# UCL/gp_emulator

Measured on AMD Instinct MI355X. Metric: test-points/sec for predict(mean+var+grad), N_train=250 D=11, higher is better.
Workload: dtype f64

## Files before the change

### gp_emulator_amd/csrc/gp_ctx.hip

```cpp
#include "gp_host.hpp"

#include <cstdarg>
#include <cstdio>

#include "gp_launchers.hpp"
#include "gp_train_args.hpp"

static thread_local char g_err[512] = "";

int fail(int code, const char* fmt, ...) {
  va_list ap;
  va_start(ap, fmt);
  vsnprintf(g_err, sizeof(g_err), fmt, ap);
  va_end(ap);
  return code;
}

int check_call(const gp_ctx* ctx, const gp_model* model, int64_t n) {
  if (!ctx || !model) return fail(GP_ERR_INVALID, "null context or model");
  if (n < 0) return fail(GP_ERR_INVALID, "n_predict < 0");
  return GP_OK;
}
int check_layout(int deriv_layout) {
  if (deriv_layout == GP_DERIV_DMAJOR || deriv_layout == GP_DERIV_ROWMAJOR) return GP_OK;
// ... 64 lines not shown
    return fail(GP_ERR_HIP, "hipStreamCreate: %s", hipGetErrorString(e));
  }
  e = hipMalloc((void**)&c->tickets, 4 * kTicketSlots * sizeof(unsigned));
  if (e == hipSuccess) e = hipMemset(c->tickets, 0, 4 * kTicketSlots * sizeof(unsigned));
  if (e != hipSuccess) {
    if (c->tickets) (void)hipFree(c->tickets);
    (void)hipStreamDestroy(c->stream);
    delete c;
    return fail(GP_ERR_HIP, "context item counters: %s", hipGetErrorString(e));
  }
  *out = c;
  return GP_OK;
}

int gp_ctx_destroy(gp_ctx* ctx) {
  if (!ctx) return GP_OK;
  (void)hipSetDevice(ctx->device);
  (void)hipStreamSynchronize(ctx->stream);
  for (auto& c : ctx->cache)
    if (c.model) gp_model_destroy(c.model);
  if (ctx->scratch) (void)hipFree(ctx->scratch);
  if (ctx->tickets) (void)hipFree(ctx->tickets);
  gp_pipe& pp = ctx->pipe;
  pp.pool.reset();
  for (int k = 0; k < kPipeSlots; ++k) {
    if (pp.stream[k]) (void)hipStreamSynchronize(pp.stream[k]);
    if (pp.stage_in[k]) (void)hipHostFree(pp.stage_in[k]);
    if (pp.stage_out[k]) (void)hipHostFree(pp.stage_out[k]);
    if (pp.dev[k]) (void)hipFree(pp.dev[k]);
    if (pp.done[k]) (void)hipEventDestroy(pp.done[k]);
    if (pp.in_there[k]) (void)hipEventDestroy(pp.in_there[k]);
    if (pp.computed[k]) (void)hipEventDestroy(pp.computed[k]);
    if (pp.stream[k]) (void)hipStreamDestroy(pp.stream[k]);
  }
  if (pp.up) { (void)hipStreamSynchronize(pp.up); (void)hipStreamDestroy(pp.up); }
  if (pp.down) { (void)hipStreamSynchronize(pp.down); (void)hipStreamDestroy(pp.down); }
  (void)hipStreamDestroy(ctx->stream);
  delete ctx;
  return GP_OK;
}

int gp_ctx_set_debug_buffer(gp_ctx* ctx, void* d_buffer) {
  if (!ctx) return fail(GP_ERR_INVALID, "null context");
  ctx->dbg = d_buffer;
  return GP_OK;
}

int gp_ctx_synchronize(gp_ctx* ctx) {
  if (!ctx) return fail(GP_ERR_INVALID, "null context");
  HIP_TRY(hipSetDevice(ctx->device));
  HIP_TRY(hipStreamSynchronize(ctx->stream));
  return GP_OK;
}

int gp_ctx_device_info(gp_ctx* ctx, int* compute_units, int64_t* hbm_bytes, char* name, int name_len) {
  if (!ctx) return fail(GP_ERR_INVALID, "null context");
// ... 148 lines not shown
```

### gp_emulator_amd/csrc/gp_host.hpp

```cpp
#pragma once
#include "gp_predict_hip.h"

#include <hip/hip_runtime.h>
#include <atomic>
#include <cstdlib>
#include <cstring>
#include <exception>
#include <memory>
#include <mutex>
#include <new>
#include <vector>

#include "gp_dispatch.hpp"
#include "gp_host_pool.hpp"
#include "gp_predict_kernel.hpp"

#pragma GCC visibility push(hidden)

int fail(int code, const char* fmt, ...) __attribute__((format(printf, 2, 3)));

template <typename F>
static int guarded(F&& body) noexcept {
  try {
    return body();
  } catch (const std::bad_alloc&) {
    return fail(GP_ERR_NOMEM, "out of host memory");
  } catch (const std::exception& ex) {
    return fail(GP_ERR_INVALID, "%s", ex.what());
  } catch (...) {
    return fail(GP_ERR_INVALID, "unknown C++ exception");
  }
}

#define HIP_TRY(expr)                                                                 \
  do {                                                                                \
    hipError_t e_ = (expr);                                                           \
    if (e_ != hipSuccess)                                                             \
// ... 21 lines not shown
template <typename T> constexpr int dtype_of() { return sizeof(T) == 8 ? GP_F64 : GP_F32; }

struct gp_model {
  int device;
  int dtype;
  int n_train, n_inputs;
  int kernel_d, kernel_nb;
  int kernel_nk;
  int n_emulators;
  long long xa_stride, frags_stride, sd_stride;
  void* d_xa;
  void* d_frags;
  void* d_sd;
  std::vector<double> scale_host, centre_host;
  std::vector<double> xs_host;
  std::mutex h_mutex;
  void* d_pfrags;
  long long pfrags_stride;
  void* d_vfrags;
  long long vfrags_stride;
};

constexpr int kPipeSlotsMax = 6;
inline int pipe_slots() {
  static const int n = [] {
    const char* ev = getenv("GP_HOST_SLOTS");
    const int v = ev ? atoi(ev) : 3;
    return v < 2 ? 2 : (v > kPipeSlotsMax ? kPipeSlotsMax : v);
  }();
  return n;
}
#define kPipeSlots pipe_slots()
struct gp_pipe {
  bool ready = false;
  hipStream_t stream[kPipeSlotsMax] = {};
  hipEvent_t done[kPipeSlotsMax] = {};
  hipStream_t up = nullptr, down = nullptr;
  hipEvent_t in_there[kPipeSlotsMax] = {}, computed[kPipeSlotsMax] = {};
  void* stage_in[kPipeSlotsMax] = {};
  void* stage_out[kPipeSlotsMax] = {};
  void* dev[kPipeSlotsMax] = {};

  size_t stage_in_bytes = 0, stage_out_bytes = 0, dev_bytes = 0;
  std::unique_ptr<gph::ThreadPool> pool;
};

struct gp_cached_model {
  gp_model* model = nullptr;
  int host_dtype = 0, compute_dtype = 0, n_train = 0, n_inputs = 0, theta_size = 0;
  bool with_invq = false;
  std::vector<char> key;
  unsigned long long stamp = 0;
};
constexpr int kModelCacheSlots = 4;

static const int kTicketSlots = 256;

struct gp_ctx {
  int device;
  hipStream_t stream;
  int compute_units;
  void* scratch;
  size_t scratch_bytes;
  void* dbg;
  unsigned* tickets = nullptr;
  std::atomic<unsigned> ticket_next{0};
  gp_pipe pipe;
// ... 51 lines not shown
```

### gp_emulator_amd/csrc/gp_host_path.hip

```cpp
#include "gp_host.hpp"

#include <cctype>
#include <chrono>
#include <cstdio>

#include <sched.h>

static int device_numa_node(int device) {
  char bdf[64] = "";
  if (hipDeviceGetPCIBusId(bdf, (int)sizeof(bdf), device) != hipSuccess) return -1;
  for (char* c = bdf; *c; ++c) *c = (char)tolower(*c);
  char path[160];
  snprintf(path, sizeof(path), "/sys/bus/pci/devices/%s/numa_node", bdf);
  FILE* fh = fopen(path, "r");
  if (!fh) return -1;
  int node = -1;
  if (fscanf(fh, "%d", &node) != 1) node = -1;
  fclose(fh);
  return node;
}
static bool node_cpus(int node, cpu_set_t* out) {
  CPU_ZERO(out);
  if (node < 0) return false;
  char path[96];
// ... 20 lines not shown
  static int n = [] {
    int avail = 1;
    cpu_set_t set;
    CPU_ZERO(&set);
    if (sched_getaffinity(0, sizeof(set), &set) == 0) avail = CPU_COUNT(&set);
    const char* ev = getenv("GP_HOST_THREADS");
    int v = ev ? atoi(ev) : 8;
    if (v > avail) v = avail;
    return v < 1 ? 1 : (v > 32 ? 32 : v);
  }();
  return n;
}

gph::ThreadPool& host_pool(gp_ctx* ctx) {
  if (!ctx->pipe.pool) {
    cpu_set_t cpus;
    const char* ev = getenv("GP_HOST_PIN");
    const bool pin = (!ev || atoi(ev) != 0) && node_cpus(device_numa_node(ctx->device), &cpus);
    ctx->pipe.pool.reset(new gph::ThreadPool(host_threads(), pin ? &cpus : nullptr));
  }
  return *ctx->pipe.pool;
}

static int ensure_pipe(gp_ctx* ctx, size_t in_bytes, size_t out_bytes, size_t dev_only_bytes = 0) {
  gp_pipe& pp = ctx->pipe;
  if (!pp.ready) {
    for (int k = 0; k < kPipeSlots; ++k) {
      if (!pp.stream[k]) HIP_TRY(hipStreamCreateWithFlags(&pp.stream[k], hipStreamNonBlocking));
      if (!pp.done[k]) HIP_TRY(hipEventCreateWithFlags(&pp.done[k], hipEventDisableTiming));
      if (!pp.in_there[k]) HIP_TRY(hipEventCreateWithFlags(&pp.in_there[k], hipEventDisableTiming));
      if (!pp.computed[k]) HIP_TRY(hipEventCreateWithFlags(&pp.computed[k], hipEventDisableTiming));
    }
    if (!pp.up) HIP_TRY(hipStreamCreateWithFlags(&pp.up, hipStreamNonBlocking));
    if (!pp.down) HIP_TRY(hipStreamCreateWithFlags(&pp.down, hipStreamNonBlocking));
    pp.ready = true;
  }
  auto host_alloc = [&](void** slot, size_t bytes) -> hipError_t {
    hipError_t err = hipSuccess;
    const int dev = ctx->device;
    host_pool(ctx).run_on_worker([&] {
      err = hipSetDevice(dev);
      if (err == hipSuccess) err = hipHostMalloc(slot, bytes, hipHostMallocDefault);
      if (err == hipSuccess) std::memset(*slot, 0, bytes);
    });
    return err;
  };
  if (dev_only_bytes == 0 && pp.stage_in_bytes < in_bytes) {
    pp.stage_in_bytes = 0;
    for (int k = 0; k < kPipeSlots; ++k) {
      if (pp.stage_in[k]) { void* q = pp.stage_in[k]; pp.stage_in[k] = nullptr; HIP_TRY(hipHostFree(q)); }
      HIP_TRY(host_alloc(&pp.stage_in[k], in_bytes));
    }
    pp.stage_in_bytes = in_bytes;
  }
  if (dev_only_bytes == 0 && pp.stage_out_bytes < out_bytes) {
    pp.stage_out_bytes = 0;
    for (int k = 0; k < kPipeSlots; ++k) {
      if (pp.stage_out[k]) { void* q = pp.stage_out[k]; pp.stage_out[k] = nullptr; HIP_TRY(hipHostFree(q)); }
      HIP_TRY(host_alloc(&pp.stage_out[k], out_bytes));
    }
    pp.stage_out_bytes = out_bytes;
  }
  const size_t dev_need = dev_only_bytes ? dev_only_bytes : in_bytes + out_bytes;
  if (pp.dev_bytes < dev_need) {
    pp.dev_bytes = 0;
    for (int k = 0; k < kPipeSlots; ++k) {
      if (pp.dev[k]) { void* q = pp.dev[k]; pp.dev[k] = nullptr; HIP_TRY(hipFree(q)); }
      HIP_TRY(hipMalloc(&pp.dev[k], dev_need));
    }
    pp.dev_bytes = dev_need;
  }
  return GP_OK;
}

template <typename T>
static int64_t slab_rows(const gp_ctx* ctx, const gp_model* m, int64_t M, int64_t out_row_elems, int64_t max_rows) {
  constexpr int64_t kRowsPerWG = gpk::Geo<T>::kRowsPerWG;
  static const int rounds = [] { const char* ev = getenv("GP_HOST_SLAB_ROUNDS"); const int v = ev ? atoi(ev) : 2; return v < 1 ? 1 : v; }();
  int64_t slab = rounds * (int64_t)ctx->compute_units * gpk::Geo<T>::kWGPerCU * kRowsPerWG;
  const int64_t by_bytes = ((int64_t)(m->n_emulators > 1 ? 64 : 16) << 20) / (int64_t)(out_row_elems * sizeof(T));
  if (slab > by_bytes) slab = by_bytes;
  if (M < 4 * slab && M >= 4 * 8192) slab = (M + 3) / 4;
  slab = (slab + kRowsPerWG - 1) / kRowsPerWG * kRowsPerWG;
  if (max_rows > 0 && slab > max_rows) slab = max_rows;
  if (slab > M) slab = M;
  return slab < 1 ? 1 : slab;
}

template <typename T, typename FIn, typename FLaunch, typename FOut>
static int run_slab_pipeline(gp_ctx* ctx, int64_t M, int64_t slab, size_t in_row, size_t out_row,
                             FIn copy_in, FLaunch launch, FOut copy_out) {
  const size_t in_elems = (size_t)slab * in_row, out_elems = (size_t)slab * out_row;
  int rc = ensure_pipe(ctx, in_elems * sizeof(T), out_elems * sizeof(T));
  if (rc) return rc;
  gp_pipe& pp = ctx->pipe;
  const int64_t ns = (M + slab - 1) / slab;
  auto rows_of = [&](int64_t s) { return (s + 1) * slab <= M ? slab : M - s * slab; };
  auto tasks_for = [&](int64_t n, size_t row_bytes) {
    const size_t bytes = (size_t)n * row_bytes;
    int t = (int)(bytes / ((size_t)256 << 10));
    const int cap = 2 * host_threads();
    return t < 1 ? 1 : (t > cap ? cap : t);
  };
  static const bool trace = [] { const char* ev = getenv("GP_HOST_TRACE"); return ev && atoi(ev) != 0; }();
  auto now = [] { return std::chrono::steady_clock::now(); };
  double t_wait = 0, t_copy = 0, t_enq = 0;
  const auto t_begin = now();
  hipError_t e = hipSuccess;
  for (int64_t s = 0; s < ns + kPipeSlots && e == hipSuccess && rc == GP_OK; ++s) {
    const int k = (int)(s % kPipeSlots);
    const int64_t so = s - kPipeSlots;
    const bool has_out = so >= 0 && so < ns, has_in = s < ns;
    if (!has_out && !has_in) continue;
    const int64_t n_out = has_out ? rows_of(so) : 0, n_in = has_in ? rows_of(s) : 0;
    auto t0 = now();
    if (has_out) {
      e = hipEventSynchronize(pp.done[k]);
      if (e != hipSuccess) break;
    }
    auto t1 = now();
    const int t_out = has_out ? tasks_for(n_out, out_row * sizeof(T)) : 0;
    const int t_in = has_in ? tasks_for(n_in, in_row * sizeof(T)) : 0;
    const T* o_stage = (const T*)pp.stage_out[k];
    T* i_stage = (T*)pp.stage_in[k];
    auto task = [&](int t) {
      if (t < t_in) {
        const int64_t lo = n_in * t / t_in, hi = n_in * (t + 1) / t_in;
        copy_in(i_stage, s * slab, n_in, lo, hi);
      } else {
        const int u = t - t_in;
        const int64_t lo = n_out * u / t_out, hi = n_out * (u + 1) / t_out;
        copy_out(o_stage, so * slab, n_out, lo, hi);
      }
    };
    const int n_tasks = t_in + t_out;
    static const int skip_host = [] { const char* ev = getenv("GP_HOST_SKIP"); return ev ? atoi(ev) & 8 : 0; }();
    if (skip_host) {}
    else if (n_tasks == 1) task(0);
    else host_pool(ctx).run(n_tasks, task);
    auto t2 = now();
    if (has_in) {
      static const int skip = [] { const char* ev = getenv("GP_HOST_SKIP"); return ev ? atoi(ev) : 0; }();
      T* d_in = (T*)pp.dev[k];
      T* d_out = d_in + in_elems;
      static const int dir_streams = [] { const char* ev = getenv("GP_PIPE_DIRSTREAMS"); return ev ? atoi(ev) : 3; }();
      const bool own_up = dir_streams & 1, own_down = dir_streams & 2;
      hipStream_t s_up = own_up ? pp.up : pp.stream[k], s_down = own_down ? pp.down : pp.stream[k];
      if (!(skip & 1))
        e = hipMemcpyAsync(d_in, pp.stage_in[k], sizeof(T) * (size_t)n_in * in_row, hipMemcpyHostToDevice, s_up);
      if (e != hipSuccess) break;
      if (own_up) {
        e = hipEventRecord(pp.in_there[k], s_up);
        if (e == hipSuccess) e = hipStreamWaitEvent(pp.stream[k], pp.in_there[k], 0);
        if (e != hipSuccess) break;
      }
      if (!(skip & 2)) rc = launch(d_in, d_out, n_in, pp.stream[k]);
      if (rc) break;
      if (own_down) {
        e = hipEventRecord(pp.computed[k], pp.stream[k]);
        if (e == hipSuccess) e = hipStreamWaitEvent(s_down, pp.computed[k], 0);
        if (e != hipSuccess) break;
      }
      if (!(skip & 4))
        e = hipMemcpyAsync(pp.stage_out[k], d_out, sizeof(T) * (size_t)n_in * out_row, hipMemcpyDeviceToHost, s_down);
      if (e == hipSuccess) e = hipEventRecord(pp.done[k], s_down);
    }
    if (trace) {
      auto t3 = now();
      t_wait += std::chrono::duration<double>(t1 - t0).count();
      t_copy += std::chrono::duration<double>(t2 - t1).count();
      t_enq += std::chrono::duration<double>(t3 - t2).count();
    }
  }
  for (int k = 0; k < kPipeSlots; ++k) (void)hipStreamSynchronize(pp.stream[k]);
  (void)hipStreamSynchronize(pp.up);
  (void)hipStreamSynchronize(pp.down);
  if (trace)
    fprintf(stderr, "[gp host pipeline] rows=%lld slab=%lld slabs=%lld threads=%d: total %.3f ms = event waits %.3f + host copies %.3f + enqueue %.3f\n",
            (long long)M, (long long)slab, (long long)ns, host_threads(),
            std::chrono::duration<double>(now() - t_begin).count() * 1e3, t_wait * 1e3, t_copy * 1e3, t_enq * 1e3);
  if (rc) return rc;
  if (e != hipSuccess) return fail(GP_ERR_HIP, "host pipeline: %s", hipGetErrorString(e));
  return GP_OK;
}

static bool is_pinned_host(const void* p, size_t bytes) {
  if (!p) return false;
  hipPointerAttribute_t a;
  if (hipPointerGetAttributes(&a, p) != hipSuccess) { (void)hipGetLastError(); return false; }
  if (a.type != hipMemoryTypeHost) return false;
  hipPointerAttribute_t b;
  if (hipPointerGetAttributes(&b, (const char*)p + (bytes ? bytes - 1 : 0)) != hipSuccess) { (void)hipGetLastError(); return false; }
  return b.type == hipMemoryTypeHost;
}

template <typename T>
static int predict_host_pinned(gp_ctx* ctx, const gp_model* m, const T* testing, T* result, T* error, T* deriv,
                               int64_t M, int64_t max_rows) {
  const int D = m->n_inputs;
  constexpr int64_t kRowsPerWG = gpk::Geo<T>::kRowsPerWG;
  const int64_t round = (int64_t)ctx->compute_units * gpk::Geo<T>::kWGPerCU * kRowsPerWG;
  int64_t cap = 4 * round;
  if (max_rows > 0 && cap > max_rows) cap = max_rows < kRowsPerWG ? kRowsPerWG : max_rows / kRowsPerWG * kRowsPerWG;
  const bool want_var = error != nullptr;
  const size_t in_elems = (size_t)cap * D, out_elems = (size_t)cap * ((want_var ? 2 : 1) + D);
  int rc = ensure_pipe(ctx, 0, 0, (in_elems + out_elems) * sizeof(T));
  if (rc) return rc;
  gp_pipe& pp = ctx->pipe;
  hipError_t e = hipSuccess;
  int64_t s0 = 0, cur = round < cap ? round : cap;
  for (int64_t s = 0; s0 < M && e == hipSuccess && rc == GP_OK; ++s) {
    const int k = (int)(s % kPipeSlots);
    const int64_t n = s0 + cur <= M ? cur : M - s0;
    if (s >= kPipeSlots) e = hipEventSynchronize(pp.done[k]);
    if (e != hipSuccess) break;
    T* d_in = (T*)pp.dev[k];
    T* d_mu = d_in + in_elems;
    T* d_var = want_var ? d_mu + n : nullptr;
    T* d_der = d_mu + (want_var ? 2 : 1) * n;
    e = hipMemcpyAsync(d_in, testing + (size_t)s0 * D, sizeof(T) * (size_t)n * D, hipMemcpyHostToDevice, pp.up);
    if (e == hipSuccess) e = hipEventRecord(pp.in_there[k], pp.up);
    if (e == hipSuccess) e = hipStreamWaitEvent(pp.stream[k], pp.in_there[k], 0);
    if (e != hipSuccess) break;
    rc = predict_device<T>(ctx, m, d_in, d_mu, d_var, d_der, n, GP_DERIV_ROWMAJOR, pp.stream[k]);
    if (rc) break;
    e = hipEventRecord(pp.computed[k], pp.stream[k]);
    if (e == hipSuccess) e = hipStreamWaitEvent(pp.down, pp.computed[k], 0);
    if (e == hipSuccess) e = hipMemcpyAsync(deriv + (size_t)s0 * D, d_der, sizeof(T) * (size_t)n * D, hipMemcpyDeviceToHost, pp.down);
    if (e == hipSuccess) e = hipMemcpyAsync(result + s0, d_mu, sizeof(T) * (size_t)n, hipMemcpyDeviceToHost, pp.down);
// ... 81 lines not shown
                             layout, st, prescale);
  };
  auto copy_out = [=](const T* o, int64_t s0, int64_t n, int64_t lo, int64_t hi) {
    int e_lo = 0, e_hi = E;
    if (E > 1) {
      e_lo = (int)((int64_t)E * lo / n);
      e_hi = (int)((int64_t)E * hi / n);
      lo = 0;
      hi = n;
    }
    for (int e = e_lo; e < e_hi; ++e) {
      convert_range(result + (size_t)e * M + s0, o + (size_t)e * n, (size_t)lo, (size_t)hi);
      if (want_var) convert_range(error + (size_t)e * M + s0, o + (size_t)(E + e) * n, (size_t)lo, (size_t)hi);
      const T* od = o + (size_t)nv * E * n + (size_t)e * n * D;
      TH* hd = deriv + (size_t)e * M * D;
      if (layout == GP_DERIV_ROWMAJOR) {
        convert_range(hd + (size_t)s0 * D, od, (size_t)lo * D, (size_t)hi * D);
      } else {
        for (int d = 0; d < D; ++d)
          convert_range(hd + (size_t)d * M + s0, od + (size_t)d * n, (size_t)lo, (size_t)hi);
      }
    }
  };
  return run_slab_pipeline<T>(ctx, M, slab, (size_t)D, out_row, copy_in, launch, copy_out);
}

template <typename T, typename TH = T>
static int hessian_host_model(gp_ctx* ctx, const gp_model* m, const TH* testing, TH* hess, int64_t M) {
  const int D = m->n_inputs, E = m->n_emulators;
  if (M == 0) return GP_OK;
  HIP_TRY(hipSetDevice(ctx->device));
  const size_t dd = (size_t)D * D;
  const size_t out_row = (size_t)E * dd;
  if (sizeof(T) == sizeof(TH) && (size_t)M * out_row * sizeof(T) <= ((size_t)8 << 20)) {
    const size_t n_in = (size_t)M * D, n_out = (size_t)M * out_row;
    int rc = ensure_scratch(ctx, (n_in + n_out) * sizeof(T));
    if (rc) return rc;
    hipStream_t st = ctx->stream;
    T* d_in = (T*)ctx->scratch;
    T* d_out = d_in + n_in;
    HIP_TRY(hipMemcpyAsync(d_in, testing, n_in * sizeof(T), hipMemcpyHostToDevice, st));
    rc = hessian_device<T>(ctx, m, d_in, d_out, M, st);
    hipError_t e = hipSuccess;
    if (!rc) e = hipMemcpyAsync(hess, d_out, n_out * sizeof(T), hipMemcpyDeviceToHost, st);
    const hipError_t es = hipStreamSynchronize(st);
    if (rc) return rc;
    if (e != hipSuccess || es != hipSuccess)
      return fail(GP_ERR_HIP, "hessian (direct copies): %s", hipGetErrorString(e != hipSuccess ? e : es));
    return GP_OK;
  }
  const int64_t slab = slab_rows<T>(ctx, m, M, (int64_t)out_row, 0);
  auto copy_in = [=](T* stage, int64_t s0, int64_t, int64_t lo, int64_t hi) {
    convert_range(stage, testing + (size_t)s0 * D, (size_t)lo * D, (size_t)hi * D);
  };
  auto launch = [=](T* d_in, T* d_out, int64_t n, hipStream_t st) {
    return hessian_device<T>(ctx, m, d_in, d_out, n, st);
  };
  auto copy_out = [=](const T* o, int64_t s0, int64_t n, int64_t lo, int64_t hi) {
    int e_lo = 0, e_hi = 1;
    if (E > 1) {
      e_lo = (int)((int64_t)E * lo / n);
      e_hi = (int)((int64_t)E * hi / n);
      lo = 0;
      hi = n;
    }
    for (int e = e_lo; e < e_hi; ++e)
      convert_range(hess + ((size_t)e * M + s0) * dd, o + (size_t)e * n * dd, (size_t)lo * dd, (size_t)hi * dd);
  };
  return run_slab_pipeline<T>(ctx, M, slab, (size_t)D, out_row, copy_in, launch, copy_out);
}

template <typename T, typename TH = T>
static int predict_wrap(gp_ctx* ctx, const TH* expX, const TH* inputs, const TH* invQt,
                        const TH* invQ, const TH* testing, TH* result, TH* error, TH* deriv,
                        int64_t M, int N, int D, int theta_size, int layout = GP_DERIV_DMAJOR) {
  if (!ctx) return fail(GP_ERR_INVALID, "null context");
  if (M < 0) return fail(GP_ERR_INVALID, "n_predict < 0");
  if (M > 0 && (!testing || !result || !error || !deriv)) return fail(GP_ERR_INVALID, "null pointer");
  if (!invQ) return fail(GP_ERR_INVALID, "null pointer");
  HIP_TRY(hipSetDevice(ctx->device));
  gp_model* m = nullptr;
  int rc = cached_model<T, TH>(ctx, expX, inputs, invQt, invQ, N, D, theta_size, &m);
  if (rc) return rc;
  return predict_host<T, TH>(ctx, m, testing, result, error, deriv, M, layout, 0);
}

template <typename T>
static int hessian_host(gp_ctx* ctx, const T* expX, const T* inputs, const T* invQt,
                        const T* testing, T* hess, int64_t M, int N, int D, int theta_size) {
  if (!ctx) return fail(GP_ERR_INVALID, "null context");
  if (M < 0) return fail(GP_ERR_INVALID, "n_predict < 0");
  if (M > 0 && (!testing || !hess)) return fail(GP_ERR_INVALID, "null pointer");
// ... 109 lines not shown
```

### gp_emulator_amd/csrc/gp_host_pool.hpp

```cpp
#pragma once
#include <atomic>
#include <condition_variable>
#include <mutex>
#include <thread>
#include <type_traits>
#include <vector>

#include <pthread.h>
#include <sched.h>

#if defined(__x86_64__)
#include <immintrin.h>
#endif

namespace gph {

inline void cpu_relax() {
#if defined(__x86_64__)
  _mm_pause();
#endif
}

class ThreadPool {
 public:
  explicit ThreadPool(int n_threads, const cpu_set_t* cpus = nullptr) {
// ... 5 lines not shown
  }
  ~ThreadPool() {
    {
      std::lock_guard<std::mutex> lk(mu_);
      stop_ = true;
      gen_.fetch_add(1, std::memory_order_release);
    }
    cv_.notify_all();
    for (auto& t : threads_) t.join();
  }
  ThreadPool(const ThreadPool&) = delete;
  ThreadPool& operator=(const ThreadPool&) = delete;

  int size() const { return (int)threads_.size() + 1; }

  template <typename F>
  void run_on_worker(F&& f) {
    if (threads_.empty()) { f(); return; }
    Job job;
    auto body = [&](int) { f(); };
    job.call = [](void* ctx, int t) { (*static_cast<decltype(body)*>(ctx))(t); };
    job.ctx = &body;
    job.n = 1;
    {
      std::lock_guard<std::mutex> lk(mu_);
      job_ = &job;
      gen_.fetch_add(1, std::memory_order_release);
    }
    cv_.notify_all();
    while (job.done.load(std::memory_order_acquire) < 1) std::this_thread::yield();
    {
      std::lock_guard<std::mutex> lk(mu_);
      job_ = nullptr;
    }
    while (job.attached.load(std::memory_order_acquire) != 0) cpu_relax();
  }

  template <typename F>
  void run(int n_tasks, F&& fn) {
    if (n_tasks <= 0) return;
    if (threads_.empty() || n_tasks == 1) {
      for (int t = 0; t < n_tasks; ++t) fn(t);
      return;
    }
    Job job;
    job.call = [](void* ctx, int t) { (*static_cast<typename std::remove_reference<F>::type*>(ctx))(t); };
    job.ctx = &fn;
    job.n = n_tasks;
    {
      std::lock_guard<std::mutex> lk(mu_);
      job_ = &job;
      gen_.fetch_add(1, std::memory_order_release);
    }
    cv_.notify_all();
    work(job);
    while (job.done.load(std::memory_order_acquire) < n_tasks) cpu_relax();
    {
      std::lock_guard<std::mutex> lk(mu_);
      job_ = nullptr;
    }
    while (job.attached.load(std::memory_order_acquire) != 0) cpu_relax();
  }

 private:
  struct Job {
    void (*call)(void*, int) = nullptr;
    void* ctx = nullptr;
    int n = 0;
    std::atomic<int> next{0}, done{0}, attached{0};
  };

  static void work(Job& job) {
    for (;;) {
      const int t = job.next.fetch_add(1, std::memory_order_relaxed);
      if (t >= job.n) break;
      job.call(job.ctx, t);
      job.done.fetch_add(1, std::memory_order_release);
    }
  }

  void worker() {
    unsigned long long seen = 0;
    for (;;) {
      for (int i = 0; i < 16000 && gen_.load(std::memory_order_acquire) == seen; ++i) cpu_relax();
      Job* job = nullptr;
      {
        std::unique_lock<std::mutex> lk(mu_);
        cv_.wait(lk, [&] { return gen_.load(std::memory_order_acquire) != seen; });
        seen = gen_.load(std::memory_order_acquire);
        if (stop_) return;
        job = job_;
        if (job) job->attached.fetch_add(1, std::memory_order_acq_rel);
      }
      if (job) {
        work(*job);
        job->attached.fetch_sub(1, std::memory_order_acq_rel);
      }
    }
  }

  std::vector<std::thread> threads_;
  std::mutex mu_;
  std::condition_variable cv_;
  std::atomic<unsigned long long> gen_{0};
  Job* job_ = nullptr;
  bool stop_ = false;
};

}
```

Measured before the change: 768.0 million.

## Decouple host staging copies from GPU slab pipeline with feeder/drainer threads

Replaces the lockstep slab loop with a staged pipeline. Dedicated feeder and drainer coordinator threads fill input staging buffers and drain output buffers independently of the main thread, which enqueues uploads, kernels and downloads on separate streams using per-slab events. The thread pool gains a job queue so several copy jobs can run at once. Input and output staging rings get independent depths. The aim is to overlap host-side copy work with transfers and kernels, at the cost of extra threads, synchronisation complexity and blocking-sync events.

```diff
diff --git a/gp_emulator_amd/csrc/gp_ctx.hip b/gp_emulator_amd/csrc/gp_ctx.hip
--- a/gp_emulator_amd/csrc/gp_ctx.hip
+++ b/gp_emulator_amd/csrc/gp_ctx.hip
@@ -110,8 +110,10 @@
   if (ctx->scratch) (void)hipFree(ctx->scratch);
   if (ctx->tickets) (void)hipFree(ctx->tickets);
   gp_pipe& pp = ctx->pipe;
+  pp.feeder.reset();
+  pp.drainer.reset();
   pp.pool.reset();
-  for (int k = 0; k < kPipeSlots; ++k) {
+  for (int k = 0; k < kPipeSlotsMax; ++k) {
     if (pp.stream[k]) (void)hipStreamSynchronize(pp.stream[k]);
     if (pp.stage_in[k]) (void)hipHostFree(pp.stage_in[k]);
     if (pp.stage_out[k]) (void)hipHostFree(pp.stage_out[k]);
@@ -120,6 +122,11 @@
     if (pp.in_there[k]) (void)hipEventDestroy(pp.in_there[k]);
     if (pp.computed[k]) (void)hipEventDestroy(pp.computed[k]);
     if (pp.stream[k]) (void)hipStreamDestroy(pp.stream[k]);
+  }
+  for (int k = 0; k < kPipeEvents; ++k) {
+    if (pp.ev_up[k]) (void)hipEventDestroy(pp.ev_up[k]);
+    if (pp.ev_kernel[k]) (void)hipEventDestroy(pp.ev_kernel[k]);
+    if (pp.ev_down[k]) (void)hipEventDestroy(pp.ev_down[k]);
   }
   if (pp.up) { (void)hipStreamSynchronize(pp.up); (void)hipStreamDestroy(pp.up); }
   if (pp.down) { (void)hipStreamSynchronize(pp.down); (void)hipStreamDestroy(pp.down); }
diff --git a/gp_emulator_amd/csrc/gp_host.hpp b/gp_emulator_amd/csrc/gp_host.hpp
--- a/gp_emulator_amd/csrc/gp_host.hpp
+++ b/gp_emulator_amd/csrc/gp_host.hpp
@@ -13,6 +13,7 @@
 
 #include "gp_dispatch.hpp"
 #include "gp_host_pool.hpp"
+#include "gp_slab_pipeline.hpp"
 #include "gp_predict_kernel.hpp"
 
 #pragma GCC visibility push(hidden)
@@ -80,14 +81,18 @@
 };
 
 constexpr int kPipeSlotsMax = 6;
+constexpr int kPipeEvents = 8;
+inline int pipe_depth_env(const char* name, int lo) {
+  const char* ev = getenv(name);
+  const int v = ev ? atoi(ev) : 3;
+  return v < lo ? lo : (v > kPipeSlotsMax ? kPipeSlotsMax : v);
+}
 inline int pipe_slots() {
-  static const int n = [] {
-    const char* ev = getenv("GP_HOST_SLOTS");
-    const int v = ev ? atoi(ev) : 3;
-    return v < 2 ? 2 : (v > kPipeSlotsMax ? kPipeSlotsMax : v);
-  }();
+  static const int n = pipe_depth_env("GP_HOST_SLOTS", 2);
   return n;
 }
+inline int pipe_ring_in() { static const int n = pipe_depth_env("GP_HOST_RING_IN", 1); return n; }
+inline int pipe_ring_out() { static const int n = pipe_depth_env("GP_HOST_RING_OUT", 1); return n; }
 #define kPipeSlots pipe_slots()
 struct gp_pipe {
   bool ready = false;
@@ -95,12 +100,15 @@
   hipEvent_t done[kPipeSlotsMax] = {};
   hipStream_t up = nullptr, down = nullptr;
   hipEvent_t in_there[kPipeSlotsMax] = {}, computed[kPipeSlotsMax] = {};
+  hipEvent_t ev_up[kPipeEvents] = {}, ev_kernel[kPipeEvents] = {}, ev_down[kPipeEvents] = {};
   void* stage_in[kPipeSlotsMax] = {};
   void* stage_out[kPipeSlotsMax] = {};
   void* dev[kPipeSlotsMax] = {};
+  int n_stage_in = 0, n_stage_out = 0;
 
   size_t stage_in_bytes = 0, stage_out_bytes = 0, dev_bytes = 0;
   std::unique_ptr<gph::ThreadPool> pool;
+  std::unique_ptr<gpsp::Coordinator> feeder, drainer;
 };
 
 struct gp_cached_model {
diff --git a/gp_emulator_amd/csrc/gp_host_path.hip b/gp_emulator_amd/csrc/gp_host_path.hip
--- a/gp_emulator_amd/csrc/gp_host_path.hip
+++ b/gp_emulator_amd/csrc/gp_host_path.hip
@@ -66,7 +66,17 @@
   return *ctx->pipe.pool;
 }
 
-static int ensure_pipe(gp_ctx* ctx, size_t in_bytes, size_t out_bytes, size_t dev_only_bytes = 0) {
+static void ensure_coordinators(gp_ctx* ctx) {
+  gp_pipe& pp = ctx->pipe;
+  if (pp.feeder && pp.drainer) return;
+  cpu_set_t cpus;
+  const char* ev = getenv("GP_HOST_PIN");
+  const bool pin = (!ev || atoi(ev) != 0) && node_cpus(device_numa_node(ctx->device), &cpus);
+  if (!pp.feeder) pp.feeder.reset(new gpsp::Coordinator(pin ? &cpus : nullptr));
+  if (!pp.drainer) pp.drainer.reset(new gpsp::Coordinator(pin ? &cpus : nullptr));
+}
+
+static int ensure_pipe(gp_ctx* ctx, size_t in_bytes, size_t out_bytes, int n_in, int n_out, size_t dev_only_bytes = 0) {
   gp_pipe& pp = ctx->pipe;
   if (!pp.ready) {
     for (int k = 0; k < kPipeSlots; ++k) {
@@ -74,6 +84,13 @@
       if (!pp.done[k]) HIP_TRY(hipEventCreateWithFlags(&pp.done[k], hipEventDisableTiming));
       if (!pp.in_there[k]) HIP_TRY(hipEventCreateWithFlags(&pp.in_there[k], hipEventDisableTiming));
       if (!pp.computed[k]) HIP_TRY(hipEventCreateWithFlags(&pp.computed[k], hipEventDisableTiming));
+    }
+    const char* ev = getenv("GP_HOST_EVENT_BLOCK");
+    const unsigned waited = hipEventDisableTiming | (!ev || atoi(ev) != 0 ? hipEventBlockingSync : 0u);
+    for (int k = 0; k < kPipeEvents; ++k) {
+      if (!pp.ev_up[k]) HIP_TRY(hipEventCreateWithFlags(&pp.ev_up[k], waited));
+      if (!pp.ev_kernel[k]) HIP_TRY(hipEventCreateWithFlags(&pp.ev_kernel[k], hipEventDisableTiming));
+      if (!pp.ev_down[k]) HIP_TRY(hipEventCreateWithFlags(&pp.ev_down[k], waited));
     }
     if (!pp.up) HIP_TRY(hipStreamCreateWithFlags(&pp.up, hipStreamNonBlocking));
     if (!pp.down) HIP_TRY(hipStreamCreateWithFlags(&pp.down, hipStreamNonBlocking));
@@ -89,21 +106,27 @@
     });
     return err;
   };
-  if (dev_only_bytes == 0 && pp.stage_in_bytes < in_bytes) {
-    pp.stage_in_bytes = 0;
-    for (int k = 0; k < kPipeSlots; ++k) {
-      if (pp.stage_in[k]) { void* q = pp.stage_in[k]; pp.stage_in[k] = nullptr; HIP_TRY(hipHostFree(q)); }
-      HIP_TRY(host_alloc(&pp.stage_in[k], in_bytes));
-    }
-    pp.stage_in_bytes = in_bytes;
-  }
-  if (dev_only_bytes == 0 && pp.stage_out_bytes < out_bytes) {
-    pp.stage_out_bytes = 0;
-    for (int k = 0; k < kPipeSlots; ++k) {
-      if (pp.stage_out[k]) { void* q = pp.stage_out[k]; pp.stage_out[k] = nullptr; HIP_TRY(hipHostFree(q)); }
-      HIP_TRY(host_alloc(&pp.stage_out[k], out_bytes));
-    }
-    pp.stage_out_bytes = out_bytes;
+  auto grow_ring = [&](void** ring, int* have, size_t* have_bytes, int want, size_t bytes) -> int {
+    if (*have_bytes < bytes) {
+      const int n = want > *have ? want : *have;
+      *have_bytes = 0;
+      *have = 0;
+      for (int k = 0; k < kPipeSlotsMax; ++k)
+        if (ring[k]) { void* q = ring[k]; ring[k] = nullptr; HIP_TRY(hipHostFree(q)); }
+      for (int k = 0; k < n; ++k) HIP_TRY(host_alloc(&ring[k], bytes));
+      *have_bytes = bytes;
+      *have = n;
+    }
+    for (int k = *have; k < want; ++k) {
+      HIP_TRY(host_alloc(&ring[k], *have_bytes));
+      *have = k + 1;
+    }
+    return GP_OK;
+  };
+  if (dev_only_bytes == 0) {
+    int rc = grow_ring(pp.stage_in, &pp.n_stage_in, &pp.stage_in_bytes, n_in, in_bytes);
+    if (!rc) rc = grow_ring(pp.stage_out, &pp.n_stage_out, &pp.stage_out_bytes, n_out, out_bytes);
+    if (rc) return rc;
   }
   const size_t dev_need = dev_only_bytes ? dev_only_bytes : in_bytes + out_bytes;
   if (pp.dev_bytes < dev_need) {
@@ -131,100 +154,144 @@
   return slab < 1 ? 1 : slab;
 }
 
+template <typename T>
+static int64_t slab_first_rows(const gp_ctx* ctx, int64_t M, int64_t slab) {
+  static const bool runup = [] { const char* ev = getenv("GP_HOST_RUNUP"); return ev && atoi(ev) != 0; }();
+  const int64_t round = (int64_t)ctx->compute_units * gpk::Geo<T>::kWGPerCU * gpk::Geo<T>::kRowsPerWG;
+  return runup && slab > round && M >= 4 * slab ? round : 0;
+}
+
+constexpr int kLaunchFailed = -(1 << 30);
+template <typename T, typename FLaunch>
+struct HipSlabBackend {
+  gp_pipe& pp;
+  const int device;
+  const size_t in_row, out_row, in_elems;
+  const std::vector<int64_t>& starts;
+  FLaunch& launch;
+  const int skip;
+  int launch_rc = GP_OK;
+
+  int64_t rows(int64_t s) const { return starts[(size_t)s + 1] - starts[(size_t)s]; }
+  static int ev(int64_t s) { return (int)(s % kPipeEvents); }
+  void thread_begin() { (void)hipSetDevice(device); }
+  int upload(int64_t s, int in_buf, int slot, int64_t after_kernel) {
+    hipError_t e = hipSuccess;
+    if (after_kernel >= 0) e = hipStreamWaitEvent(pp.up, pp.ev_kernel[ev(after_kernel)], 0);
+    if (e == hipSuccess && !(skip & 1))
+      e = hipMemcpyAsync(pp.dev[slot], pp.stage_in[in_buf], sizeof(T) * (size_t)rows(s) * in_row, hipMemcpyHostToDevice, pp.up);
+    if (e == hipSuccess) e = hipEventRecord(pp.ev_up[ev(s)], pp.up);
+    return (int)e;
+  }
+  int kernel(int64_t s, int slot, int64_t after_download) {
+    hipStream_t st = pp.stream[slot];
+    hipError_t e = hipStreamWaitEvent(st, pp.ev_up[ev(s)], 0);
+    if (e == hipSuccess && after_download >= 0) e = hipStreamWaitEvent(st, pp.ev_down[ev(after_download)], 0);
+    if (e != hipSuccess) return (int)e;
+    T* d_in = (T*)pp.dev[slot];
+    if (!(skip & 2) && (launch_rc = launch(d_in, d_in + in_elems, rows(s), st))) return kLaunchFailed;
+    return (int)hipEventRecord(pp.ev_kernel[ev(s)], st);
+  }
+  int download(int64_t s, int slot, int out_buf) {
+    hipError_t e = hipStreamWaitEvent(pp.down, pp.ev_kernel[ev(s)], 0);
+    if (e == hipSuccess && !(skip & 4))
+      e = hipMemcpyAsync(pp.stage_out[out_buf], (T*)pp.dev[slot] + in_elems, sizeof(T) * (size_t)rows(s) * out_row,
+                         hipMemcpyDeviceToHost, pp.down);
+    if (e == hipSuccess) e = hipEventRecord(pp.ev_down[ev(s)], pp.down);
+    return (int)e;
+  }
+  int wait_upload(int64_t s) { return (int)hipEventSynchronize(pp.ev_up[ev(s)]); }
+  int wait_download(int64_t s) { return (int)hipEventSynchronize(pp.ev_down[ev(s)]); }
+  static int query(hipEvent_t e) {
+    const hipError_t q = hipEventQuery(e);
+    if (q == hipSuccess) return 1;
+    if (q == hipErrorNotReady) { (void)hipGetLastError(); return 0; }
+    return -(int)q;
+  }
+  int upload_done(int64_t s) { return query(pp.ev_up[ev(s)]); }
+  int download_done(int64_t s) { return query(pp.ev_down[ev(s)]); }
+  void drain() {
+    for (int k = 0; k < kPipeSlots; ++k) (void)hipStreamSynchronize(pp.stream[k]);
+    (void)hipStreamSynchronize(pp.up);
+    (void)hipStreamSynchronize(pp.down);
+  }
+};
+
 template <typename T, typename FIn, typename FLaunch, typename FOut>
-static int run_slab_pipeline(gp_ctx* ctx, int64_t M, int64_t slab, size_t in_row, size_t out_row,
+static int run_slab_pipeline(gp_ctx* ctx, int64_t M, int64_t slab, int64_t first, size_t in_row, size_t out_row,
                              FIn copy_in, FLaunch launch, FOut copy_out) {
   const size_t in_elems = (size_t)slab * in_row, out_elems = (size_t)slab * out_row;
-  int rc = ensure_pipe(ctx, in_elems * sizeof(T), out_elems * sizeof(T));
+  std::vector<int64_t> starts{0};
+  if (first > 0 && first < slab && first < M) starts.push_back(first);
+  while (starts.back() < M) starts.push_back(starts.back() + slab < M ? starts.back() + slab : M);
+  const int64_t ns = (int64_t)starts.size() - 1;
+  static const size_t cap = [] { const char* ev = getenv("GP_HOST_STAGE_CAP_MB"); const long v = ev ? atol(ev) : 256; return (size_t)(v < 1 ? 1 : v) << 20; }();
+  auto depth = [&](int want, size_t bytes) {
+    int dpt = want;
+    while (dpt > 1 && (size_t)dpt * bytes > cap) --dpt;
+    return (int64_t)dpt > ns ? (int)ns : dpt;
+  };
+  gpsp::Depths depths;
+  depths.s_in = depth(pipe_ring_in(), in_elems * sizeof(T));
+  depths.s_out = depth(pipe_ring_out(), out_elems * sizeof(T));
+  depths.s_dev = kPipeSlots;
+  int rc = ensure_pipe(ctx, in_elems * sizeof(T), out_elems * sizeof(T), depths.s_in, depths.s_out);
   if (rc) return rc;
   gp_pipe& pp = ctx->pipe;
-  const int64_t ns = (M + slab - 1) / slab;
-  auto rows_of = [&](int64_t s) { return (s + 1) * slab <= M ? slab : M - s * slab; };
-  auto tasks_for = [&](int64_t n, size_t row_bytes) {
-    const size_t bytes = (size_t)n * row_bytes;
-    int t = (int)(bytes / ((size_t)256 << 10));
-    const int cap = 2 * host_threads();
-    return t < 1 ? 1 : (t > cap ? cap : t);
-  };
+  static const bool coordinators = [] { const char* ev = getenv("GP_HOST_COORD"); return !ev || atoi(ev) != 0; }();
+  if (coordinators) ensure_coordinators(ctx);
+  static const int skip = [] { const char* ev = getenv("GP_HOST_SKIP"); return ev ? atoi(ev) : 0; }();
   static const bool trace = [] { const char* ev = getenv("GP_HOST_TRACE"); return ev && atoi(ev) != 0; }();
-  auto now = [] { return std::chrono::steady_clock::now(); };
-  double t_wait = 0, t_copy = 0, t_enq = 0;
-  const auto t_begin = now();
-  hipError_t e = hipSuccess;
-  for (int64_t s = 0; s < ns + kPipeSlots && e == hipSuccess && rc == GP_OK; ++s) {
-    const int k = (int)(s % kPipeSlots);
-    const int64_t so = s - kPipeSlots;
-    const bool has_out = so >= 0 && so < ns, has_in = s < ns;
-    if (!has_out && !has_in) continue;
-    const int64_t n_out = has_out ? rows_of(so) : 0, n_in = has_in ? rows_of(s) : 0;
-    auto t0 = now();
-    if (has_out) {
-      e = hipEventSynchronize(pp.done[k]);
-      if (e != hipSuccess) break;
-    }
-    auto t1 = now();
-    const int t_out = has_out ? tasks_for(n_out, out_row * sizeof(T)) : 0;
-    const int t_in = has_in ? tasks_for(n_in, in_row * sizeof(T)) : 0;
-    const T* o_stage = (const T*)pp.stage_out[k];
-    T* i_stage = (T*)pp.stage_in[k];
-    auto task = [&](int t) {
-      if (t < t_in) {
-        const int64_t lo = n_in * t / t_in, hi = n_in * (t + 1) / t_in;
-        copy_in(i_stage, s * slab, n_in, lo, hi);
-      } else {
-        const int u = t - t_in;
-        const int64_t lo = n_out * u / t_out, hi = n_out * (u + 1) / t_out;
-        copy_out(o_stage, so * slab, n_out, lo, hi);
-      }
-    };
-    const int n_tasks = t_in + t_out;
-    static const int skip_host = [] { const char* ev = getenv("GP_HOST_SKIP"); return ev ? atoi(ev) & 8 : 0; }();
-    if (skip_host) {}
-    else if (n_tasks == 1) task(0);
-    else host_pool(ctx).run(n_tasks, task);
-    auto t2 = now();
-    if (has_in) {
-      static const int skip = [] { const char* ev = getenv("GP_HOST_SKIP"); return ev ? atoi(ev) : 0; }();
-      T* d_in = (T*)pp.dev[k];
-      T* d_out = d_in + in_elems;
-      static const int dir_streams = [] { const char* ev = getenv("GP_PIPE_DIRSTREAMS"); return ev ? atoi(ev) : 3; }();
-      const bool own_up = dir_streams & 1, own_down = dir_streams & 2;
-      hipStream_t s_up = own_up ? pp.up : pp.stream[k], s_down = own_down ? pp.down : pp.stream[k];
-      if (!(skip & 1))
-        e = hipMemcpyAsync(d_in, pp.stage_in[k], sizeof(T) * (size_t)n_in * in_row, hipMemcpyHostToDevice, s_up);
-      if (e != hipSuccess) break;
-      if (own_up) {
-        e = hipEventRecord(pp.in_there[k], s_up);
-        if (e == hipSuccess) e = hipStreamWaitEvent(pp.stream[k], pp.in_there[k], 0);
-        if (e != hipSuccess) break;
-      }
-      if (!(skip & 2)) rc = launch(d_in, d_out, n_in, pp.stream[k]);
-      if (rc) break;
-      if (own_down) {
-        e = hipEventRecord(pp.computed[k], pp.stream[k]);
-        if (e == hipSuccess) e = hipStreamWaitEvent(s_down, pp.computed[k], 0);
-        if (e != hipSuccess) break;
-      }
-      if (!(skip & 4))
-        e = hipMemcpyAsync(pp.stage_out[k], d_out, sizeof(T) * (size_t)n_in * out_row, hipMemcpyDeviceToHost, s_down);
-      if (e == hipSuccess) e = hipEventRecord(pp.done[k], s_down);
-    }
-    if (trace) {
-      auto t3 = now();
-      t_wait += std::chrono::duration<double>(t1 - t0).count();
-      t_copy += std::chrono::duration<double>(t2 - t1).count();
-      t_enq += std::chrono::duration<double>(t3 - t2).count();
-    }
-  }
-  for (int k = 0; k < kPipeSlots; ++k) (void)hipStreamSynchronize(pp.stream[k]);
-  (void)hipStreamSynchronize(pp.up);
-  (void)hipStreamSynchronize(pp.down);
+
+  struct HostSide {
+    const std::vector<int64_t>& starts;
+    gp_pipe& pp;
+    FIn& copy_in;
+    FOut& copy_out;
+    size_t in_bytes_row, out_bytes_row;
+    bool skip_copies;
+    int64_t rows(int64_t s) const { return starts[(size_t)s + 1] - starts[(size_t)s]; }
+    static int tasks_for(int64_t n, size_t row_bytes) {
+      const size_t bytes = (size_t)n * row_bytes;
+      const int t = (int)(bytes / ((size_t)256 << 10));
+      const int cap = 2 * host_threads();
+      return t < 1 ? 1 : (t > cap ? cap : t);
+    }
+    int in_tasks(int64_t s) const { return tasks_for(rows(s), in_bytes_row); }
+    int out_tasks(int64_t s) const { return tasks_for(rows(s), out_bytes_row); }
+    void copy_in_task(int64_t s, int buf, int t, int n_tasks) {
+      if (skip_copies) return;
+      const int64_t n = rows(s);
+      copy_in((T*)pp.stage_in[buf], starts[(size_t)s], n, n * t / n_tasks, n * (t + 1) / n_tasks);
+    }
+    void copy_out_task(int64_t s, int buf, int t, int n_tasks) {
+      if (skip_copies) return;
+      const int64_t n = rows(s);
+      copy_out((const T*)pp.stage_out[buf], starts[(size_t)s], n, n * t / n_tasks, n * (t + 1) / n_tasks);
+    }
+  };
+  struct HostAdapter {
+    HostSide& h;
+    int in_tasks(int64_t s) const { return h.in_tasks(s); }
+    int out_tasks(int64_t s) const { return h.out_tasks(s); }
+    void copy_in(int64_t s, int buf, int t, int n) { h.copy_in_task(s, buf, t, n); }
+    void copy_out(int64_t s, int buf, int t, int n) { h.copy_out_task(s, buf, t, n); }
+  };
+  HostSide side{starts, pp, copy_in, copy_out, in_row * sizeof(T), out_row * sizeof(T), (skip & 8) != 0};
+  HostAdapter host{side};
+  HipSlabBackend<T, FLaunch> be{pp, ctx->device, in_row, out_row, in_elems, starts, launch, skip};
+  gpsp::Stats tm;
+  rc = gpsp::run_slabs(be, host, host_pool(ctx), coordinators ? pp.feeder.get() : nullptr,
+                       coordinators ? pp.drainer.get() : nullptr, ns, depths, trace ? &tm : nullptr);
   if (trace)
-    fprintf(stderr, "[gp host pipeline] rows=%lld slab=%lld slabs=%lld threads=%d: total %.3f ms = event waits %.3f + host copies %.3f + enqueue %.3f\n",
-            (long long)M, (long long)slab, (long long)ns, host_threads(),
-            std::chrono::duration<double>(now() - t_begin).count() * 1e3, t_wait * 1e3, t_copy * 1e3, t_enq * 1e3);
-  if (rc) return rc;
-  if (e != hipSuccess) return fail(GP_ERR_HIP, "host pipeline: %s", hipGetErrorString(e));
+    fprintf(stderr, "[gp host pipeline] rows=%lld slab=%lld first=%lld slabs=%lld threads=%d rings=%d/%d/%d %s: total %.3f ms; "
+            "caller: blocked on copy-in %.3f + blocked on output buffer %.3f + enqueue %.3f; "
+            "feeder: copying %.3f + waiting for the device %.3f; drainer: copying %.3f + waiting for the device %.3f\n",
+            (long long)M, (long long)slab, (long long)starts[1], (long long)ns, host_threads(), depths.s_in, depths.s_dev,
+            depths.s_out, coordinators ? "coordinators" : "polling", tm.total * 1e3, tm.blocked_in * 1e3, tm.blocked_out * 1e3,
+            tm.enqueue * 1e3, tm.feeder_copy * 1e3, tm.feeder_wait * 1e3, tm.drainer_copy * 1e3, tm.drainer_wait * 1e3);
+  if (rc == kLaunchFailed) return be.launch_rc;
+  if (rc) return fail(GP_ERR_HIP, "host pipeline: %s", hipGetErrorString((hipError_t)(rc < 0 ? -rc : rc)));
   return GP_OK;
 }
 
@@ -248,7 +315,7 @@
   if (max_rows > 0 && cap > max_rows) cap = max_rows < kRowsPerWG ? kRowsPerWG : max_rows / kRowsPerWG * kRowsPerWG;
   const bool want_var = error != nullptr;
   const size_t in_elems = (size_t)cap * D, out_elems = (size_t)cap * ((want_var ? 2 : 1) + D);
-  int rc = ensure_pipe(ctx, 0, 0, (in_elems + out_elems) * sizeof(T));
+  int rc = ensure_pipe(ctx, 0, 0, 0, 0, (in_elems + out_elems) * sizeof(T));
   if (rc) return rc;
   gp_pipe& pp = ctx->pipe;
   hipError_t e = hipSuccess;
@@ -376,7 +443,7 @@
       }
     }
   };
-  return run_slab_pipeline<T>(ctx, M, slab, (size_t)D, out_row, copy_in, launch, copy_out);
+  return run_slab_pipeline<T>(ctx, M, slab, slab_first_rows<T>(ctx, M, slab), (size_t)D, out_row, copy_in, launch, copy_out);
 }
 
 template <typename T, typename TH = T>
@@ -421,7 +488,7 @@
     for (int e = e_lo; e < e_hi; ++e)
       convert_range(hess + ((size_t)e * M + s0) * dd, o + (size_t)e * n * dd, (size_t)lo * dd, (size_t)hi * dd);
   };
-  return run_slab_pipeline<T>(ctx, M, slab, (size_t)D, out_row, copy_in, launch, copy_out);
+  return run_slab_pipeline<T>(ctx, M, slab, slab_first_rows<T>(ctx, M, slab), (size_t)D, out_row, copy_in, launch, copy_out);
 }
 
 template <typename T, typename TH = T>
diff --git a/gp_emulator_amd/csrc/gp_host_pool.hpp b/gp_emulator_amd/csrc/gp_host_pool.hpp
--- a/gp_emulator_amd/csrc/gp_host_pool.hpp
+++ b/gp_emulator_amd/csrc/gp_host_pool.hpp
@@ -1,6 +1,7 @@
 #pragma once
 #include <atomic>
 #include <condition_variable>
+#include <deque>
 #include <mutex>
 #include <thread>
 #include <type_traits>
@@ -52,18 +53,9 @@
     job.call = [](void* ctx, int t) { (*static_cast<decltype(body)*>(ctx))(t); };
     job.ctx = &body;
     job.n = 1;
-    {
-      std::lock_guard<std::mutex> lk(mu_);
-      job_ = &job;
-      gen_.fetch_add(1, std::memory_order_release);
-    }
-    cv_.notify_all();
+    push(job);
     while (job.done.load(std::memory_order_acquire) < 1) std::this_thread::yield();
-    {
-      std::lock_guard<std::mutex> lk(mu_);
-      job_ = nullptr;
-    }
-    while (job.attached.load(std::memory_order_acquire) != 0) cpu_relax();
+    retire(job);
   }
 
   template <typename F>
@@ -77,19 +69,29 @@
     job.call = [](void* ctx, int t) { (*static_cast<typename std::remove_reference<F>::type*>(ctx))(t); };
     job.ctx = &fn;
     job.n = n_tasks;
-    {
-      std::lock_guard<std::mutex> lk(mu_);
-      job_ = &job;
-      gen_.fetch_add(1, std::memory_order_release);
-    }
-    cv_.notify_all();
+    push(job);
     work(job);
     while (job.done.load(std::memory_order_acquire) < n_tasks) cpu_relax();
-    {
-      std::lock_guard<std::mutex> lk(mu_);
-      job_ = nullptr;
+    retire(job);
+  }
+
+  template <typename P>
+  void help_until(P&& done) {
+    std::unique_lock<std::mutex> lk(mu_);
+    for (;;) {
+      if (done()) return;
+      Job* job = claimable();
+      if (!job) { cv_.wait(lk); continue; }
+      job->attached.fetch_add(1, std::memory_order_acq_rel);
+      lk.unlock();
+      while (work_one(*job) && !done()) {}
+      job->attached.fetch_sub(1, std::memory_order_acq_rel);
+      lk.lock();
     }
-    while (job.attached.load(std::memory_order_acquire) != 0) cpu_relax();
+  }
+  void notify() {
+    { std::lock_guard<std::mutex> lk(mu_); }
+    cv_.notify_all();
   }
 
  private:
@@ -100,28 +102,54 @@
     std::atomic<int> next{0}, done{0}, attached{0};
   };
 
+  void push(Job& job) {
+    {
+      std::lock_guard<std::mutex> lk(mu_);
+      queue_.push_back(&job);
+      gen_.fetch_add(1, std::memory_order_release);
+    }
+    cv_.notify_all();
+  }
+  void retire(Job& job) {
+    {
+      std::lock_guard<std::mutex> lk(mu_);
+      for (size_t i = 0; i < queue_.size(); ++i)
+        if (queue_[i] == &job) { queue_.erase(queue_.begin() + (long)i); break; }
+    }
+    while (job.attached.load(std::memory_order_acquire) != 0) cpu_relax();
+  }
+  Job* claimable() const {
+    for (Job* j : queue_)
+      if (j->next.load(std::memory_order_relaxed) < j->n) return j;
+    return nullptr;
+  }
+
+  static bool work_one(Job& job) {
+    const int t = job.next.fetch_add(1, std::memory_order_relaxed);
+    if (t >= job.n) return false;
+    job.call(job.ctx, t);
+    job.done.fetch_add(1, std::memory_order_release);
+    return true;
+  }
   static void work(Job& job) {
-    for (;;) {
-      const int t = job.next.fetch_add(1, std::memory_order_relaxed);
-      if (t >= job.n) break;
-      job.call(job.ctx, t);
-      job.done.fetch_add(1, std::memory_order_release);
-    }
+    while (work_one(job)) {}
   }
 
   void worker() {
     unsigned long long seen = 0;
+    bool again = false;
     for (;;) {
-      for (int i = 0; i < 16000 && gen_.load(std::memory_order_acquire) == seen; ++i) cpu_relax();
+      for (int i = 0; !again && i < 16000 && gen_.load(std::memory_order_acquire) == seen; ++i) cpu_relax();
       Job* job = nullptr;
       {
         std::unique_lock<std::mutex> lk(mu_);
-        cv_.wait(lk, [&] { return gen_.load(std::memory_order_acquire) != seen; });
+        if (!again) cv_.wait(lk, [&] { return stop_ || gen_.load(std::memory_order_acquire) != seen; });
+        if (stop_) return;
         seen = gen_.load(std::memory_order_acquire);
-        if (stop_) return;
-        job = job_;
+        job = claimable();
         if (job) job->attached.fetch_add(1, std::memory_order_acq_rel);
       }
+      again = job != nullptr;
       if (job) {
         work(*job);
         job->attached.fetch_sub(1, std::memory_order_acq_rel);
@@ -133,7 +161,7 @@
   std::mutex mu_;
   std::condition_variable cv_;
   std::atomic<unsigned long long> gen_{0};
-  Job* job_ = nullptr;
+  std::deque<Job*> queue_;
   bool stop_ = false;
 };
 
diff --git a/gp_emulator_amd/csrc/gp_slab_pipeline.hpp b/gp_emulator_amd/csrc/gp_slab_pipeline.hpp
--- /dev/null
+++ b/gp_emulator_amd/csrc/gp_slab_pipeline.hpp
@@ -0,0 +1,231 @@
+#pragma once
+#include <atomic>
+#include <chrono>
+#include <condition_variable>
+#include <cstdint>
+#include <functional>
+#include <mutex>
+#include <thread>
+
+#include "gp_host_pool.hpp"
+
+namespace gpsp {
+
+struct Depths {
+  int s_in = 3, s_dev = 3, s_out = 3;
+};
+
+struct Stats {
+  double total = 0;
+  double blocked_in = 0, blocked_out = 0, enqueue = 0;
+  double feeder_copy = 0, feeder_wait = 0;
+  double drainer_copy = 0, drainer_wait = 0;
+};
+
+class Coordinator {
+ public:
+  explicit Coordinator(const cpu_set_t* cpus = nullptr) : th_([this] { loop(); }) {
+    if (cpus) (void)pthread_setaffinity_np(th_.native_handle(), sizeof(cpu_set_t), cpus);
+  }
+  ~Coordinator() {
+    {
+      std::lock_guard<std::mutex> lk(mu_);
+      stop_ = true;
+    }
+    cv_.notify_all();
+    th_.join();
+  }
+  Coordinator(const Coordinator&) = delete;
+  Coordinator& operator=(const Coordinator&) = delete;
+
+  void start(std::function<void()> f) {
+    {
+      std::lock_guard<std::mutex> lk(mu_);
+      fn_ = std::move(f);
+      busy_ = true;
+    }
+    cv_.notify_all();
+  }
+  void wait() {
+    std::unique_lock<std::mutex> lk(mu_);
+    cv_.wait(lk, [&] { return !busy_; });
+  }
+
+ private:
+  void loop() {
+    std::unique_lock<std::mutex> lk(mu_);
+    for (;;) {
+      cv_.wait(lk, [&] { return stop_ || fn_; });
+      if (stop_) return;
+      std::function<void()> f = std::move(fn_);
+      fn_ = nullptr;
+      lk.unlock();
+      f();
+      lk.lock();
+      busy_ = false;
+      cv_.notify_all();
+    }
+  }
+  std::mutex mu_;
+  std::condition_variable cv_;
+  std::function<void()> fn_;
+  bool busy_ = false, stop_ = false;
+  std::thread th_;
+};
+
+namespace detail {
+using clock = std::chrono::steady_clock;
+inline double since(clock::time_point t0) { return std::chrono::duration<double>(clock::now() - t0).count(); }
+
+struct State {
+  std::atomic<int64_t> fed{0}, drained{0}, up{0}, down{0};
+  std::atomic<int> err{0};
+  std::mutex mu;
+  std::condition_variable cv;
+};
+}
+
+template <typename Backend, typename Host>
+int run_slabs(Backend& be, Host& host, gph::ThreadPool& pool, Coordinator* feeder, Coordinator* drainer,
+              int64_t ns, Depths d, Stats* stats = nullptr) {
+  using namespace detail;
+  if (ns <= 0) return 0;
+  const int64_t S_in = d.s_in < 1 ? 1 : d.s_in, S_dev = d.s_dev < 1 ? 1 : d.s_dev, S_out = d.s_out < 1 ? 1 : d.s_out;
+  const bool threads = feeder && drainer;
+  const auto t_begin = clock::now();
+  State st;
+  Stats tm;
+  auto wake = [&] {
+    { std::lock_guard<std::mutex> lk(st.mu); }
+    st.cv.notify_all();
+  };
+  auto set_err = [&](int rc) {
+    int none = 0;
+    st.err.compare_exchange_strong(none, rc);
+    wake();
+    pool.notify();
+  };
+  auto failed = [&] { return st.err.load(std::memory_order_acquire) != 0; };
+  auto feed = [&](int64_t s) {
+    const int n = host.in_tasks(s), buf = (int)(s % S_in);
+    const auto t0 = clock::now();
+    pool.run(n, [&](int t) { host.copy_in(s, buf, t, n); });
+    tm.feeder_copy += since(t0);
+    st.fed.store(s + 1, std::memory_order_release);
+  };
+  auto drain_slab = [&](int64_t s) {
+    const int n = host.out_tasks(s), buf = (int)(s % S_out);
+    const auto t0 = clock::now();
+    pool.run(n, [&](int t) { host.copy_out(s, buf, t, n); });
+    tm.drainer_copy += since(t0);
+    st.drained.store(s + 1, std::memory_order_release);
+  };
+
+  if (threads) {
+    feeder->start([&] {
+      be.thread_begin();
+      for (int64_t s = 0; s < ns && !failed(); ++s) {
+        const int64_t u = s - S_in;
+        if (u >= 0) {
+          const auto t0 = clock::now();
+          {
+            std::unique_lock<std::mutex> lk(st.mu);
+            st.cv.wait(lk, [&] { return failed() || st.up.load(std::memory_order_acquire) > u; });
+          }
+          if (failed()) break;
+          const int rc = be.wait_upload(u);
+          tm.feeder_wait += since(t0);
+          if (rc) { set_err(rc); break; }
+        }
+        feed(s);
+        pool.notify();
+      }
+    });
+    drainer->start([&] {
+      be.thread_begin();
+      for (int64_t s = 0; s < ns && !failed(); ++s) {
+        const auto t0 = clock::now();
+        {
+          std::unique_lock<std::mutex> lk(st.mu);
+          st.cv.wait(lk, [&] { return failed() || st.down.load(std::memory_order_acquire) > s; });
+        }
+        if (failed()) break;
+        const int rc = be.wait_download(s);
+        tm.drainer_wait += since(t0);
+        if (rc) { set_err(rc); break; }
+        drain_slab(s);
+        pool.notify();
+      }
+    });
+  }
+
+  int64_t next_up = 0, next_down = 0;
+  auto can_down = [&] {
+    return next_down < next_up && st.drained.load(std::memory_order_acquire) > next_down - S_out;
+  };
+  auto can_up = [&] {
+    return next_up < ns && next_up < next_down + S_dev && st.fed.load(std::memory_order_acquire) > next_up;
+  };
+  while (next_down < ns && !failed()) {
+    if (can_down() || can_up()) {
+      const auto t0 = clock::now();
+      int rc = 0;
+      if (can_down()) {
+        const int64_t s = next_down;
+        rc = be.download(s, (int)(s % S_dev), (int)(s % S_out));
+        if (!rc) st.down.store(++next_down, std::memory_order_release);
+      } else {
+        const int64_t s = next_up, before = s - S_dev >= 0 ? s - S_dev : -1;
+        rc = be.upload(s, (int)(s % S_in), (int)(s % S_dev), before);
+        if (!rc) rc = be.kernel(s, (int)(s % S_dev), before);
+        if (!rc) st.up.store(++next_up, std::memory_order_release);
+      }
+      if (rc) set_err(rc);
+      else if (threads) wake();
+      tm.enqueue += since(t0);
+      continue;
+    }
+    const bool for_in = next_up < ns && next_up < next_down + S_dev;
+    const auto t0 = clock::now();
+    if (threads) {
+      pool.help_until([&] { return failed() || can_down() || can_up(); });
+    } else {
+      const int64_t f = st.fed.load(std::memory_order_relaxed), u = f - S_in;
+      const int64_t o = st.drained.load(std::memory_order_relaxed);
+      int fin = f < ns ? (u < 0 ? 1 : (u < next_up ? be.upload_done(u) : 0)) : 0;
+      int fout = o < next_down ? be.download_done(o) : 0;
+      int rc = 0;
+      if (fin == 0 && fout == 0) {
+        if (o < next_down) { rc = be.wait_download(o); fout = 1; }
+        else { rc = be.wait_upload(u); fin = 1; }
+      }
+      if (rc || fin < 0 || fout < 0) { set_err(rc ? rc : (fin < 0 ? fin : fout)); break; }
+      if (fout > 0) drain_slab(o);
+      if (fin > 0) feed(f);
+    }
+    (for_in ? tm.blocked_in : tm.blocked_out) += since(t0);
+  }
+  {
+    const auto t0 = clock::now();
+    if (threads) {
+      pool.help_until([&] { return failed() || st.drained.load(std::memory_order_acquire) >= ns; });
+    } else {
+      for (int64_t o = st.drained.load(std::memory_order_relaxed); o < ns && !failed(); ++o) {
+        const int rc = be.wait_download(o);
+        if (rc) { set_err(rc); break; }
+        drain_slab(o);
+      }
+    }
+    tm.blocked_out += since(t0);
+  }
+  if (threads) {
+    feeder->wait();
+    drainer->wait();
+  }
+  be.drain();
+  tm.total = since(t_begin);
+  if (stats) *stats = tm;
+  return st.err.load(std::memory_order_acquire);
+}
+
+}
```

Result: no change. 767.8 million (-0.0%).
